# lucidrains/audiolm-pytorch

Hardware: NVIDIA H100
Metric: CoarseTransformer tokens/sec fwd+bwd seq2048 (higher is better)
Workload: dtype bf16

## Files before the change

### audiolm_pytorch_b200/_lib.py

```python
from __future__ import annotations

import ctypes as C
import os
from pathlib import Path

import torch

_PKG = Path(__file__).resolve().parent
LIB_PATH = _PKG / "libalm_b200.so"

P = C.c_void_p
I = C.c_int
L = C.c_int64
F = C.c_float
U32 = C.c_uint32
U64 = C.c_uint64
DROP = [F, U64, U32]

SIGNATURES: dict[str, list] = {
    "alm_gemm_bf16": [P, I, L, L, P, I, L, L, P, I, L, L, I, I, I, I, F, P, I, I, P],
    "alm_mqa_attn_fwd": [P, L, P, L, L, P, L, L, P, P, L, P, L, P, L, L, I, I, I, I, I, F, *DROP, P],
    "alm_mqa_attn_bwd": [P, L, P, L, L, P, L, L, P, L, P, P, P, I, P, L, P, P, L, P, L, P, P, L, L, I, I, I, I, I, F, *DROP,
                         P],
    "alm_pack_key_mask": [P, P, I, I, P],
# ... 22 lines not shown
    "alm_cast_pad_multi": [P, I, P],
    "alm_scale_by_scalar_bf16": [P, P, L, P],
    "alm_topk_gumbel_sample": [P, L, P, L, P, I, I, I, F, P],
    "alm_resid_ln_fwd": [P, P, P, P, P, P, P, I, I, P],
    "alm_resid_ln_bwd": [P, P, P, P, P, P, P, P, P, F, I, I, P],
    "alm_residual_unit_fwd": [P, P, P, P, P, P, I, I, I, I, I, P],
    "alm_causal_conv1d_fwd": [P, P, P, P, P, I, I, I, I, I, I, I, I, I, I, P],
    "alm_causal_convT1d_fwd": [P, P, P, P, I, I, I, I, I, P],
    "alm_codec_first_conv": [P, P, P, P, I, I, I, I, I, P],
    "alm_codec_ru_tc": [P, P, P, P, P, I, I, I, I, I, I, P],
    "alm_codec_conv_tc": [P, P, P, P, I, I, I, I, I, I, I, I, I, I, P],
    "alm_codec_pack_c8s": [P, P, I, I, I, P],
    "alm_codec_last_conv": [P, P, P, P, I, I, I, I, I, P],
    "alm_rvq_encode": [P, L, P, P, P, L, P, L, I, I, I, I, P],
    "alm_rvq_pack_codebooks": [P, P, P, L, I, P],
    "alm_rvq_prepare": [P, L, P, P, L, P, I, I, P],
    "alm_rvq_select": [P, L, P, P, P, P, L, P, P, L, I, I, I, I, P],
    "alm_rvq_decode": [P, L, P, P, L, I, I, I, I, P],
}


class AlmError(RuntimeError):
    pass


_lib = None


def load() -> C.CDLL:
    global _lib
    if _lib is not None:
        return _lib
    if not LIB_PATH.exists():
        raise AlmError(
            f"{LIB_PATH} not found. Build it with `python -m audiolm_pytorch_b200.build` "
            "(there is no CPU / PyTorch fallback for the hot path)."
        )
    lib = C.CDLL(str(LIB_PATH), mode=os.RTLD_LOCAL | os.RTLD_NOW)
    lib.alm_version.restype = I
    lib.alm_status_string.restype = C.c_char_p
    lib.alm_status_string.argtypes = [I]
    lib.alm_launch_count.restype = C.c_ulonglong
    lib.alm_reset_launch_count.restype = None
    lib.alm_decode_stack_scratch_bytes.restype = L
    lib.alm_decode_stack_scratch_bytes.argtypes = [I, I, I, I]
    lib.alm_gemm_head_ce_tiles.restype = I
    lib.alm_gemm_head_ce_tiles.argtypes = [I]
    lib.alm_decode_stack_grid.restype = I
    lib.alm_decode_stack_grid.argtypes = []
    lib.alm_decode_stack_plan.restype = I
    lib.alm_decode_stack_plan.argtypes = [I, I, I, I, I, P]
    lib.alm_decode_stack_trace_offset.restype = L
    lib.alm_decode_stack_trace_offset.argtypes = [I, I, I, I]
    for name, argtypes in SIGNATURES.items():
        fn = getattr(lib, name)
        fn.argtypes = argtypes
        fn.restype = I
    _lib = lib
    return lib


def ptr(t) -> int | None:
    if t is None:
        return None
    return t.data_ptr()


def stream_handle() -> int:
    return torch.cuda.current_stream().cuda_stream


def call(name: str, *args) -> None:
    lib = load()
    conv = []
    for a in args:
        if isinstance(a, torch.Tensor):
            if not a.is_cuda:
                raise AlmError(f"{name}: got a {a.device} tensor; the hot path has no CPU implementation")
            conv.append(a.data_ptr())
        else:
            conv.append(a)
    rc = getattr(lib, name)(*conv, stream_handle())
    if rc != 0:
        raise AlmError(f"{name} failed: {lib.alm_status_string(rc).decode()} ({rc})")


def launch_count() -> int:
    return int(load().alm_launch_count())


def reset_launch_count() -> None:
    load().alm_reset_launch_count()
```

### audiolm_pytorch_b200/csrc/attn_fwd_wgmma.cu

```cuda
#include "alm_common.cuh"
#include "ptx_sm90.cuh"

namespace alm {

constexpr int ATT_BM = 128;
constexpr int ATT_BN = 128;
constexpr int ATT_D = 64;
constexpr int ATT_KV_STAGES = 4;
constexpr int ATT_THREADS = 384;
constexpr int ATT_TILE_BYTES = 128 * 64 * 2;
constexpr int ATT_SMEM_BYTES = ATT_TILE_BYTES * (1 + 2 * ATT_KV_STAGES) + 256;

struct AttnFwdParams {
  __nv_bfloat16* o;
  float* lse;
  const uint32_t* kmask;
  int kb_stride;
  const float* bias;
  long long bias_hs, bias_rs;
  long long ldo, lse_stride;
  int b, h, n_q, n_k;
  int causal;
  float scale_log2;
  int n_q_pad;
  DropoutArgs drop;
};

__device__ __forceinline__ float att_ex2(float x) {
  float y;
  asm("ex2.approx.ftz.f32 %0, %1;" : "=f"(y) : "f"(x));
  return y;
}

__device__ __forceinline__ uint64_t attn_fwd_keep_bits(const DropoutArgs& d, uint32_t qrow, uint32_t kbase, int c_lane) {
  const uint32_t odd = qrow & 1u;
  uint64_t bits = 0;
#pragma unroll
  for (int kk = 0; kk < ATT_BN / 16; ++kk) {
    const uint32_t j0 = kbase + 16 * kk + c_lane;
    const uint4 own = dropout_draw(d, qrow, j0 + odd);
    const uint32_t ra = __shfl_xor_sync(0xffffffffu, odd ? own.x : own.y, 4);
    const uint32_t rb = __shfl_xor_sync(0xffffffffu, odd ? own.z : own.w, 4);
    const uint4 other = odd ? make_uint4(0u, ra, 0u, rb) : make_uint4(ra, 0u, rb, 0u);
#pragma unroll
    for (int c = 0; c < 2; ++c) {
      const uint4 dr = (uint32_t)c == odd ? own : other;
#pragma unroll
      for (int half = 0; half < 2; ++half)
#pragma unroll
        for (int h = 0; h < 2; ++h)
          if (dropout_pick(d, dr, qrow + 8 * h, j0 + 8 * half + c)) bits |= 1ull << (8 * kk + 4 * half + 2 * h + c);
    }
  }
  return bits;
}

template <bool HAS_BIAS, bool DROPOUT>
__global__ void __launch_bounds__(ATT_THREADS, 1)
mqa_attn_fwd_kernel(const __grid_constant__ CUtensorMap tmQ, const __grid_constant__ CUtensorMap tmK,
                    const __grid_constant__ CUtensorMap tmV, const AttnFwdParams p) {
  extern __shared__ __align__(1024) uint8_t smem_raw[];
  uint8_t* smem = smem_raw;
  if ((smem_u32(smem) & 1023u) != 0) __trap();
  uint8_t* sQ = smem;
  uint8_t* sK = sQ + ATT_TILE_BYTES;
  uint8_t* sV = sK + ATT_KV_STAGES * ATT_TILE_BYTES;
  uint64_t* bars = reinterpret_cast<uint64_t*>(sV + ATT_KV_STAGES * ATT_TILE_BYTES);
  uint64_t* q_full = bars;
  uint64_t* kv_full = bars + 1;
  uint64_t* kv_empty = kv_full + ATT_KV_STAGES;

  const int warp = threadIdx.x >> 5;
  const int lane = threadIdx.x & 31;
  const int wg = warp >> 2;
  const int n_qblocks = (p.n_q + ATT_BM - 1) / ATT_BM;
  const int qb = n_qblocks - 1 - (int)blockIdx.x;
  const int head = blockIdx.y;
  const int batch = blockIdx.z;
  const int q0 = qb * ATT_BM;
  const int off = p.n_k - p.n_q;
  int kv_end = p.n_k;
  if (p.causal) kv_end = min(p.n_k, q0 + ATT_BM + off);
  const int n_tiles = kv_end > 0 ? (kv_end + ATT_BN - 1) / ATT_BN : 0;

  if (threadIdx.x == 0) {
    tma_prefetch_desc(&tmQ);
    tma_prefetch_desc(&tmK);
    tma_prefetch_desc(&tmV);
    mbar_init(q_full, 1);
    for (int i = 0; i < ATT_KV_STAGES; ++i) {
      mbar_init(&kv_full[i], 1);
      mbar_init(&kv_empty[i], 8);
    }
    fence_mbar_init();
  }
  __syncthreads();

  if (wg == 0) {
    if (warp == 0 && n_tiles > 0) {
      if (elect_one_sync()) {
        mbar_arrive_expect_tx(q_full, ATT_TILE_BYTES);
        tma_load_3d(sQ, &tmQ, q_full, head * ATT_D, q0, batch);
      }
      __syncwarp();
      int stage = 0;
      uint32_t phase = 0;
      for (int j = 0; j < n_tiles; ++j) {
        mbar_wait(&kv_empty[stage], phase ^ 1u);
        if (elect_one_sync()) {
          mbar_arrive_expect_tx(&kv_full[stage], 2 * ATT_TILE_BYTES);
          tma_load_3d(sK + stage * ATT_TILE_BYTES, &tmK, &kv_full[stage], 0, j * ATT_BN, batch);
          tma_load_3d(sV + stage * ATT_TILE_BYTES, &tmV, &kv_full[stage], 0, j * ATT_BN, batch);
        }
        __syncwarp();
        if (++stage == ATT_KV_STAGES) { stage = 0; phase ^= 1u; }
      }
    }
    return;
  }

  const int cw = wg - 1;
  const int r_base = cw * 64 + (warp & 3) * 16 + (lane >> 2);
  const int c_lane = 2 * (lane & 3);
  constexpr float kLog2e = 1.4426950408889634f;
  float m_run[2] = {-INFINITY, -INFINITY}, l_run[2] = {0.f, 0.f};
  float o_acc[ATT_D / 2];
#pragma unroll
  for (int d = 0; d < ATT_D / 2; ++d) o_acc[d] = 0.f;
  int q_limit[2];
  [[maybe_unused]] const float* brow[2];
#pragma unroll
  for (int h = 0; h < 2; ++h) {
    const int qi = q0 + r_base + 8 * h;
    q_limit[h] = min(p.causal ? qi + off : p.n_k - 1, p.n_k - 1);
    if constexpr (HAS_BIAS) brow[h] = p.bias + (long long)head * p.bias_hs + (long long)min(qi, p.n_q - 1) * p.bias_rs;
  }
  const uint32_t* mrow = p.kmask ? p.kmask + (long long)batch * p.kb_stride : nullptr;
  const uint32_t q_addr = smem_u32(sQ) + cw * 8192;
  [[maybe_unused]] const uint32_t drop_row = ((uint32_t)batch * p.h + head) * (uint32_t)p.n_q_pad + q0 + r_base;

  if (n_tiles > 0) mbar_wait(q_full, 0);
  int stage = 0;
  uint32_t phase = 0;
  for (int j = 0; j < n_tiles; ++j) {
    mbar_wait(&kv_full[stage], phase);
    const uint32_t k_addr = smem_u32(sK + stage * ATT_TILE_BYTES);
    const uint32_t v_addr = smem_u32(sV + stage * ATT_TILE_BYTES);
    float s[ATT_BN / 2];
    wgmma_fence();
#pragma unroll
    for (int k = 0; k < ATT_D / 16; ++k)
      wgmma_ss<ATT_BN>(s, wgmma_desc_sw128(q_addr + k * 32, 1024, 16), wgmma_desc_sw128(k_addr + k * 32, 1024, 16),
                       k > 0 ? 1u : 0u);
    wgmma_commit();
    [[maybe_unused]] uint64_t keep = 0;
    if constexpr (DROPOUT) keep = attn_fwd_keep_bits(p.drop, drop_row, j * ATT_BN, c_lane);
    wgmma_wait<0>();
    wgmma_fence_acc(s);

    const int kbase = j * ATT_BN;
    const bool tile_full = mrow == nullptr && kbase + ATT_BN <= p.n_k && (!p.causal || kbase + ATT_BN - 1 <= q0 + off);
    uint32_t valid[4] = {0xFFFFFFFFu, 0xFFFFFFFFu, 0xFFFFFFFFu, 0xFFFFFFFFu};
    if (!tile_full && mrow != nullptr) {
      const uint4 mv = __ldg(reinterpret_cast<const uint4*>(mrow + j * 4));
      valid[0] = mv.x; valid[1] = mv.y; valid[2] = mv.z; valid[3] = mv.w;
    }
    uint32_t pa[ATT_BN / 16][4];
#pragma unroll
    for (int h = 0; h < 2; ++h) {
#pragma unroll
      for (int g = 0; g < ATT_BN / 8; ++g)
#pragma unroll
        for (int c = 0; c < 2; ++c) {
          const int col = 8 * g + c_lane + c;
          float v = s[4 * g + 2 * h + c] * p.scale_log2;
          if constexpr (HAS_BIAS) {
            if (kbase + col < p.bias_rs) v = fmaf(__ldg(brow[h] + kbase + col), kLog2e, v);
          }
          if (!tile_full) {
            const bool ok = kbase + col <= q_limit[h] && ((valid[col >> 5] >> (col & 31)) & 1u);
            if (!ok) v = -INFINITY;
          }
          s[4 * g + 2 * h + c] = v;
        }
      float m_tile = -INFINITY;
#pragma unroll
      for (int g = 0; g < ATT_BN / 8; ++g) m_tile = fmaxf(m_tile, fmaxf(s[4 * g + 2 * h], s[4 * g + 2 * h + 1]));
      m_tile = fmaxf(m_tile, __shfl_xor_sync(0xffffffffu, m_tile, 1));
      m_tile = fmaxf(m_tile, __shfl_xor_sync(0xffffffffu, m_tile, 2));
      const float m_new = fmaxf(m_run[h], m_tile);
      const float m_use = (m_new == -INFINITY) ? 0.f : m_new;
      const float alpha = att_ex2(m_run[h] - m_use);
      float l_tile = 0.f;
#pragma unroll
      for (int g = 0; g < ATT_BN / 8; ++g)
#pragma unroll
        for (int c = 0; c < 2; ++c) {
          const float pv = att_ex2(s[4 * g + 2 * h + c] - m_use);
          s[4 * g + 2 * h + c] = pv;
          l_tile += pv;
        }
      l_run[h] = fmaf(l_run[h], alpha, l_tile);
      m_run[h] = m_new;
#pragma unroll
      for (int g = 0; g < ATT_D / 8; ++g) {
        o_acc[4 * g + 2 * h] *= alpha;
        o_acc[4 * g + 2 * h + 1] *= alpha;
      }
    }
    if constexpr (DROPOUT) {
#pragma unroll
      for (int e = 0; e < ATT_BN / 2; ++e) s[e] = ((keep >> e) & 1u) ? s[e] * p.drop.scale : 0.f;
    }
#pragma unroll
    for (int kk = 0; kk < ATT_BN / 16; ++kk) {
      pa[kk][0] = pack_bf16x2(s[8 * kk + 0], s[8 * kk + 1]);
      pa[kk][1] = pack_bf16x2(s[8 * kk + 2], s[8 * kk + 3]);
      pa[kk][2] = pack_bf16x2(s[8 * kk + 4], s[8 * kk + 5]);
      pa[kk][3] = pack_bf16x2(s[8 * kk + 6], s[8 * kk + 7]);
    }
    wgmma_fence_acc(o_acc);
    wgmma_fence();
#pragma unroll
    for (int kk = 0; kk < ATT_BN / 16; ++kk)
      wgmma_rs<ATT_D, 1>(o_acc, pa[kk], wgmma_desc_sw128(v_addr + kk * 2048, 1024, 8192), 1u);
    wgmma_commit();
    wgmma_wait<0>();
    wgmma_fence_acc(o_acc);
    if (lane == 0) mbar_arrive(&kv_empty[stage]);
    if (++stage == ATT_KV_STAGES) { stage = 0; phase ^= 1u; }
  }

#pragma unroll
  for (int h = 0; h < 2; ++h) {
    float l_tot = l_run[h];
    l_tot += __shfl_xor_sync(0xffffffffu, l_tot, 1);
    l_tot += __shfl_xor_sync(0xffffffffu, l_tot, 2);
    const int qi = q0 + r_base + 8 * h;
    if (qi < p.n_q) {
      const float inv = l_tot > 0.f ? 1.f / l_tot : 0.f;
      __nv_bfloat16* dst = p.o + ((long long)batch * p.n_q + qi) * p.ldo + head * ATT_D + c_lane;
#pragma unroll
      for (int g = 0; g < ATT_D / 8; ++g)
        *reinterpret_cast<uint32_t*>(dst + 8 * g) = pack_bf16x2(o_acc[4 * g + 2 * h] * inv, o_acc[4 * g + 2 * h + 1] * inv);
      if (p.lse != nullptr && (lane & 3) == 0) {
        const float lse = l_tot > 0.f ? (m_run[h] + log2f(l_tot)) : INFINITY;
        p.lse[((long long)batch * p.h + head) * p.lse_stride + qi] = lse;
      }
    }
  }
}

}

namespace alm {
__global__ void pack_key_mask_kernel(const uint8_t* __restrict__ mask, uint32_t* __restrict__ bits, int n_k, int words) {
  const int b = blockIdx.y;
  const int w = blockIdx.x * (blockDim.x >> 5) + (threadIdx.x >> 5);
  if (w >= words) return;
  const int k = w * 32 + (threadIdx.x & 31);
  const bool on = k < n_k && mask[(long long)b * n_k + k] != 0;
  const uint32_t v = __ballot_sync(0xffffffffu, on);
  if ((threadIdx.x & 31) == 0) bits[(long long)b * words + w] = v;
}
}

extern "C" int alm_pack_key_mask(const void* key_mask, void* bits, int b, int n_k, alm_stream_t stream_) {
  using namespace alm;
  cudaStream_t stream = reinterpret_cast<cudaStream_t>(stream_);
  ALM_REQUIRE(key_mask && bits && b > 0 && n_k > 0, ALM_ERR_ARG);
  const int words = (n_k + 127) / 128 * 4;
  dim3 grid(ceil_div(words, 8), b);
  pack_key_mask_kernel<<<grid, 256, 0, stream>>>(reinterpret_cast<const uint8_t*>(key_mask),
                                                 reinterpret_cast<uint32_t*>(bits), n_k, words);
  ALM_CHECK_LAUNCH();
  ALM_LAUNCHED(1);
  return ALM_OK;
}

extern "C" int alm_mqa_attn_fwd(const void* q, int64_t ldq, const void* k, int64_t ldk, int64_t k_bstride,
                                const void* v, int64_t ldv, int64_t v_bstride, const void* key_mask, void* o,
                                int64_t ldo, float* lse, int64_t lse_stride, const float* bias, int64_t bias_hstride,
                                int64_t bias_rstride, int b, int h, int n_q, int n_k, int causal, float scale,
                                float dropout_p, uint64_t seed, uint32_t site, alm_stream_t stream_) {
  using namespace alm;
  cudaStream_t stream = reinterpret_cast<cudaStream_t>(stream_);
  ALM_REQUIRE(q && k && v && o, ALM_ERR_ARG);
  ALM_REQUIRE(b > 0 && h > 0 && n_q > 0 && n_k > 0 && n_k >= n_q, ALM_ERR_ARG);
  ALM_REQUIRE(dropout_p >= 0.f && dropout_p < 1.f, ALM_ERR_ARG);
  ALM_REQUIRE((long long)b * h * ((n_q + 127) / 128 * 128) < (1ll << 32), ALM_ERR_UNSUPPORTED);
  ALM_REQUIRE(ldq % 8 == 0 && ldk % 8 == 0 && ldv % 8 == 0 && ldo % 8 == 0, ALM_ERR_ALIGN);
  ALM_REQUIRE(k_bstride % 8 == 0 && v_bstride % 8 == 0, ALM_ERR_ALIGN);
  ALM_REQUIRE((reinterpret_cast<uintptr_t>(o) & 15u) == 0, ALM_ERR_ALIGN);
  if (bias != nullptr) {
    ALM_REQUIRE(bias_rstride >= n_k && bias_rstride % 4 == 0 && bias_hstride % 4 == 0, ALM_ERR_ALIGN);
    ALM_REQUIRE((reinterpret_cast<uintptr_t>(bias) & 15u) == 0, ALM_ERR_ALIGN);
  }

  CUtensorMap tmQ, tmK, tmV;
  {
    uint64_t dims[3] = {(uint64_t)h * ATT_D, (uint64_t)n_q, (uint64_t)b};
    uint64_t strides[3] = {2, (uint64_t)ldq * 2, (uint64_t)n_q * ldq * 2};
    uint32_t box[3] = {ATT_D, ATT_BM, 1};
    int rc = make_tensor_map(&tmQ, q, 2, 3, dims, strides, box, true);
    if (rc != ALM_OK) return rc;
  }
  {
    uint64_t dims[3] = {(uint64_t)ATT_D, (uint64_t)n_k, (uint64_t)b};
    uint64_t strides[3] = {2, (uint64_t)ldk * 2, (uint64_t)k_bstride * 2};
    uint32_t box[3] = {ATT_D, ATT_BN, 1};
    int rc = make_tensor_map(&tmK, k, 2, 3, dims, strides, box, true);
    if (rc != ALM_OK) return rc;
    strides[1] = (uint64_t)ldv * 2;
    strides[2] = (uint64_t)v_bstride * 2;
    rc = make_tensor_map(&tmV, v, 2, 3, dims, strides, box, true);
    if (rc != ALM_OK) return rc;
  }
  AttnFwdParams p;
  p.o = reinterpret_cast<__nv_bfloat16*>(o);
  p.lse = lse;
  p.kmask = reinterpret_cast<const uint32_t*>(key_mask);
  p.kb_stride = (n_k + 127) / 128 * 4;
  p.bias = bias;
  p.bias_hs = bias_hstride;
  p.bias_rs = bias_rstride;
  p.ldo = ldo;
  p.lse_stride = lse_stride;
  p.b = b; p.h = h; p.n_q = n_q; p.n_k = n_k;
  p.causal = causal;
  p.scale_log2 = scale * 1.4426950408889634f;
  p.n_q_pad = (n_q + 127) / 128 * 128;
  p.drop = make_dropout_args(dropout_p, seed, site);
  static bool attr_set = false;
  if (!attr_set) {
    ALM_CUDA_OK(cudaFuncSetAttribute(mqa_attn_fwd_kernel<false, false>, cudaFuncAttributeMaxDynamicSharedMemorySize,
                                     ATT_SMEM_BYTES));
    ALM_CUDA_OK(cudaFuncSetAttribute(mqa_attn_fwd_kernel<true, false>, cudaFuncAttributeMaxDynamicSharedMemorySize,
                                     ATT_SMEM_BYTES));
    ALM_CUDA_OK(cudaFuncSetAttribute(mqa_attn_fwd_kernel<false, true>, cudaFuncAttributeMaxDynamicSharedMemorySize,
                                     ATT_SMEM_BYTES));
    ALM_CUDA_OK(cudaFuncSetAttribute(mqa_attn_fwd_kernel<true, true>, cudaFuncAttributeMaxDynamicSharedMemorySize,
                                     ATT_SMEM_BYTES));
    attr_set = true;
  }
  dim3 grid((n_q + ATT_BM - 1) / ATT_BM, h, b);
  const bool drop = dropout_p > 0.f;
  if (bias != nullptr && drop)
    mqa_attn_fwd_kernel<true, true><<<grid, ATT_THREADS, ATT_SMEM_BYTES, stream>>>(tmQ, tmK, tmV, p);
  else if (bias != nullptr)
    mqa_attn_fwd_kernel<true, false><<<grid, ATT_THREADS, ATT_SMEM_BYTES, stream>>>(tmQ, tmK, tmV, p);
  else if (drop)
    mqa_attn_fwd_kernel<false, true><<<grid, ATT_THREADS, ATT_SMEM_BYTES, stream>>>(tmQ, tmK, tmV, p);
  else
    mqa_attn_fwd_kernel<false, false><<<grid, ATT_THREADS, ATT_SMEM_BYTES, stream>>>(tmQ, tmK, tmV, p);
  ALM_CHECK_LAUNCH();
  ALM_LAUNCHED(1);
  return ALM_OK;
}
```

### audiolm_pytorch_b200/ops.py

```python
from __future__ import annotations

import ctypes
import functools

import torch

from . import _lib

_SMS: dict[int, int] = {}


def num_sms(device=None) -> int:
    idx = None if device is None else torch.device(device).index
    if idx is None:
        idx = torch.cuda.current_device()
    if idx not in _SMS:
        _SMS[idx] = torch.cuda.get_device_properties(idx).multi_processor_count
    return _SMS[idx]


bf16 = torch.bfloat16
f32 = torch.float32


# ... 134 lines not shown
    bits = torch.empty(b, (n_k + 127) // 128 * 4, device=m.device, dtype=torch.int32)
    _lib.call("alm_pack_key_mask", m, bits, b, n_k)
    return PackedKeyMask(bits, n_k)


def _drop_args(dropout):
    if dropout is None:
        return 0.0, 0, 0
    p, seed, site = dropout
    if not 0.0 <= p < 1.0:
        raise ValueError(f"dropout probability must be in [0, 1), got {p}")
    return float(p), int(seed) & 0xFFFFFFFFFFFFFFFF, int(site) & 0xFFFFFFFF


def dropout_(x, p, seed, site):
    _check_cuda(x)
    assert x.dtype == bf16 and x.dim() == 2 and x.stride(1) == 1
    M, C = x.shape
    with _timed("dropout_bf16", M * C * 4, "byte"):
        _lib.call("alm_dropout_bf16", x, x.stride(0), M, C, *_drop_args((p, seed, site)))
    return x


def mqa_attn_fwd(q, k, v, *, heads, key_mask=None, causal=True, scale=None, return_lse=True, bias=None,
                 dropout=None):
    _check_cuda(q, k, v, bias)
    assert q.dtype == bf16 and k.dtype == bf16 and v.dtype == bf16
    b, n_q, hd = q.shape
    n_k = k.shape[1]
    assert hd == heads * 64 and k.shape[-1] == 64 and v.shape[-1] == 64, "dim_head must be 64"
    assert q.stride(-1) == 1 and k.stride(-1) == 1 and v.stride(-1) == 1
    assert q.stride(0) == n_q * q.stride(1)
    o = torch.empty(b, n_q, hd, device=q.device, dtype=bf16)
    n_q_pad = (n_q + 127) // 128 * 128
    lse = torch.empty(b, heads, n_q_pad, device=q.device, dtype=f32) if return_lse else None
    key_mask = pack_key_mask(key_mask)
    if key_mask is not None:
        assert key_mask.n_k == n_k and key_mask.bits.shape[0] == b
        key_mask = key_mask.bits
    if scale is None:
        scale = 64 ** -0.5
    vis = (n_q * n_k - n_q * (n_q - 1) / 2) if causal else n_q * n_k
    bhs, brs = _check_bias(bias, heads, n_q, n_k) if bias is not None else (0, 0)
    with _timed("mqa_attn_fwd_wgmma", 4.0 * b * heads * 64 * vis):
        _lib.call(
            "alm_mqa_attn_fwd",
            q, q.stride(1), k, k.stride(1), k.stride(0), v, v.stride(1), v.stride(0), key_mask,
            o, o.stride(1), lse, n_q_pad, bias, bhs, brs, b, heads, n_q, n_k, int(causal), float(scale),
            *_drop_args(dropout),
        )
    return o, lse


def mqa_attn_bwd(q, k, v, o, d_o, lse, *, heads, key_mask=None, causal=True, scale=None, bias=None, dbias=None,
                 dropout=None):
    _check_cuda(q, k, v, o, d_o, lse, bias, dbias)
    b, n_q, hd = q.shape
    n_k = k.shape[1]
    n_q_pad = lse.shape[-1]
    assert d_o.dtype == bf16 and d_o.stride(-1) == 1 and o.stride(-1) == 1
    assert d_o.stride(0) == n_q * d_o.stride(1)
    key_mask = pack_key_mask(key_mask)
    if key_mask is not None:
        assert key_mask.n_k == n_k
        key_mask = key_mask.bits
    if scale is None:
        scale = 64 ** -0.5
    dq = torch.empty(b, n_q, hd, device=q.device, dtype=bf16)
    delta = torch.empty(b, heads, n_q_pad, device=q.device, dtype=f32)
    dq_acc = torch.empty(b, n_q, hd, device=q.device, dtype=f32)
    dk = torch.empty(b, n_k, 64, device=q.device, dtype=bf16)
    dv = torch.empty(b, n_k, 64, device=q.device, dtype=bf16)
    bhs, brs = _check_bias(bias, heads, n_q, n_k) if bias is not None else (0, 0)
    if dbias is not None:
        assert bias is not None and dbias.dtype == f32 and dbias.shape == bias.shape and dbias.stride() == bias.stride()
    vis = (n_q * n_k - n_q * (n_q - 1) / 2) if causal else n_q * n_k
    with _timed("mqa_attn_bwd_wgmma", 10.0 * b * heads * 64 * vis):
        _lib.call("alm_attn_delta", o, o.stride(1), d_o, d_o.stride(1), delta, n_q_pad, dq_acc, b, heads, n_q)
        _lib.call(
            "alm_mqa_attn_bwd",
            q, q.stride(1), k, k.stride(1), k.stride(0), v, v.stride(1), v.stride(0), d_o, d_o.stride(1), key_mask,
            lse, delta, n_q_pad, dq, dq.stride(1), dq_acc, dk, dk.stride(1), dv, dv.stride(1),
            bias, dbias, bhs, brs, b, heads, n_q, n_k, int(causal), float(scale), *_drop_args(dropout),
        )
    return dq, dk, dv


def gemv(x, w, *, out_dtype=bf16, bias=None):
    _check_cuda(x, w, bias)
    rows, K = x.shape
    N = w.shape[0]
    assert x.dtype == bf16 and w.dtype == bf16 and x.stride(1) == 1 and w.stride(1) == 1 and rows <= 8
    assert w.shape[1] >= K and w.shape[1] % 8 == 0
    out = torch.empty(rows, N, device=x.device, dtype=out_dtype)
    _lib.call("alm_gemv_bf16", x, x.stride(0), w, w.stride(0), out, int(out_dtype == f32), out.stride(0),
              None if bias is None else bias.float().contiguous(), rows, N, K)
    return out


def kv_append(kv_new, k_cache, v_cache, cache_len):
    _check_cuda(kv_new, k_cache, v_cache, cache_len)
    b, max_len, dh = k_cache.shape
    assert dh == 64 and v_cache.shape == k_cache.shape and kv_new.shape == (b, 128) and kv_new.dtype == bf16
    assert k_cache.dtype == bf16 and v_cache.dtype == bf16 and cache_len.dtype == torch.int32
    assert k_cache.stride(1) == 64 and v_cache.stride() == k_cache.stride() and kv_new.stride(1) == 1
    _lib.call("alm_kv_append", kv_new, kv_new.stride(0), k_cache, v_cache, k_cache.stride(0), cache_len, max_len, b)
# ... 526 lines not shown
```

### include/alm_b200.h

```cpp
#ifndef ALM_B200_H_
#define ALM_B200_H_

#include <stddef.h>
#include <stdint.h>

#ifdef __cplusplus
extern "C" {
#endif

typedef struct CUstream_st* alm_stream_t;

typedef enum alm_status {
  ALM_OK = 0,
  ALM_ERR_ARG = -1,
  ALM_ERR_ALIGN = -2,
  ALM_ERR_CUDA = -3,
  ALM_ERR_UNSUPPORTED = -4
} alm_status;

int alm_version(void);
const char* alm_status_string(int code);
unsigned long long alm_launch_count(void);
void alm_reset_launch_count(void);

int alm_gemm_bf16(const void* A, int a_mn, int64_t lda, int64_t strideA, const void* B, int b_mn, int64_t ldb,
                  int64_t strideB, void* C, int c_fp32, int64_t ldc, int64_t strideC, int M, int N, int K, int batch,
                  float alpha, const float* bias, int acc_mode, int split_k, alm_stream_t stream);

int alm_embed_gather(const float* const* tables, int n_tables, const int32_t* src, float* out, int M, int d,
                     alm_stream_t stream);
int alm_embed_scatter(float* const* grad_tables, int n_tables, const int32_t* src, const float* dout, int M, int d,
                      alm_stream_t stream);
int alm_pack_key_mask(const void* key_mask, void* bits, int b, int n_k, alm_stream_t stream);
int alm_mqa_attn_fwd(const void* q, int64_t ldq, const void* k, int64_t ldk, int64_t k_bstride, const void* v,
                     int64_t ldv, int64_t v_bstride, const void* key_mask, void* o, int64_t ldo, float* lse,
                     int64_t lse_stride, const float* bias, int64_t bias_hstride, int64_t bias_rstride, int b, int h,
                     int n_q, int n_k, int causal, float scale, float dropout_p, uint64_t seed, uint32_t site,
                     alm_stream_t stream);

int alm_mqa_attn_bwd(const void* q, int64_t ldq, const void* k, int64_t ldk, int64_t k_bstride, const void* v,
                     int64_t ldv, int64_t v_bstride, const void* d_o, int64_t lddo, const void* key_mask,
                     const float* lse, const float* delta, int n_q_pad, void* dq, int64_t lddq, float* dq_acc,
                     void* dk, int64_t lddk, void* dv, int64_t lddv, const float* bias, float* dbias,
                     int64_t bias_hstride, int64_t bias_rstride, int b, int h, int n_q, int n_k, int causal,
                     float scale, float dropout_p, uint64_t seed, uint32_t site, alm_stream_t stream);
int alm_attn_delta(const void* o, int64_t ldo, const void* d_o, int64_t lddo, float* delta ,
                   int64_t delta_stride, float* dq_acc, int b, int h, int n, alm_stream_t stream);

int alm_bias_gather_fwd(const float* table, const int32_t* idx, const float* override_h, float* out, int heads,
                        int n_q, int n_k, int64_t ld, alm_stream_t stream);
int alm_bias_gather_bwd(const float* dbias, const int32_t* idx, float* dtable, float* doverride, int heads, int n_q,
                        int n_k, int64_t ld, alm_stream_t stream);

int alm_gemv_bf16(const void* x, int64_t ldx, const void* W, int64_t ldw, void* out, int c_fp32, int64_t ldo,
                  const float* bias, int rows, int N, int K, alm_stream_t stream);
int alm_kv_append(const void* kv_new, int64_t ld, void* k_cache, void* v_cache, int64_t cache_bstride,
                  const int32_t* len, int max_len, int b, alm_stream_t stream);
int alm_mqa_attn_decode(const void* q, int64_t ldq, const void* k_cache, const void* v_cache, int64_t cache_bstride,
                        const int32_t* len, int max_len, const void* key_mask, int64_t mask_bstride, const float* bias,
                        int64_t bias_ld, void* o, int64_t ldo,
                        float* workspace , int splits, int b, int h,
                        float scale, alm_stream_t stream);
int alm_decode_bias_row(const float* table, int rows, const float* override_h, const int32_t* u, const int32_t* cls,
                        int c, const int32_t* len, int max_len, float* out, int64_t ld, int h, alm_stream_t stream);

int alm_gemm_head_ce_tiles(int V);
int alm_gemm_head_ce(const void* X, int64_t ldx, const void* W, int64_t ldw, const float* bias, const int64_t* labels,
                     int64_t ignore_index, int mode, float* part, float* lab_logit, const float* lse,
                     const float* scale_num, const float* scale_den, void* dlogits, int64_t ldd, int M, int V, int K,
                     alm_stream_t stream);
int alm_ce_finish(const float* part, int tiles, const float* lab_logit, const int64_t* labels, int64_t ignore_index,
                  float* lse, float* loss_rows, int M, alm_stream_t stream);

int alm_decode_stack_grid(void);
int alm_decode_stack_plan(int b, int d, int heads, int inner, int n_layers, int32_t* staged);
int64_t alm_decode_stack_scratch_bytes(int b, int d, int heads, int inner);
int64_t alm_decode_stack_trace_offset(int b, int d, int heads, int inner);
int alm_decode_stack_step(const void* layer_table, int n_layers, const float* x, void* out, const float* final_gamma,
                          int32_t* len, int max_len, int64_t cache_bstride, const void* key_mask, int64_t mask_bstride,
                          void* scratch, int64_t scratch_bytes, int b, int d, int heads, int inner, int value_residual,
                          float scale, int grid_ctas , alm_stream_t stream);

int alm_hc_pre_fwd(const void* R_in, const void* Y, const float* beta_prev, const float* x_expand,
                   const float* gamma_hc, const float* dyn_alpha, const float* dyn_beta, const float* static_alpha,
                   const float* static_beta, const float* alpha_scale, const float* beta_scale,
                   const float* ln_gamma, void* R_out, void* bin, void* xn, float* beta_out, float* aux, int M,
                   int d, int streams, alm_stream_t stream);
int alm_hc_pre_bwd(const void* R_in, const void* Y, const float* beta_prev, const float* x_expand,
                   const float* gamma_hc, const float* dyn_alpha, const float* dyn_beta, const float* static_alpha,
                   const float* static_beta, const float* alpha_scale, const float* beta_scale,
                   const float* ln_gamma, const float* aux, const void* dR_out, const void* dxn,
// ... 74 lines not shown
```

Measured before the change: 746,100.

## Make attention forward persistent with double-buffered Q and S/PV wgmma overlap

Turns the attention forward kernel into a persistent kernel. A grid sized to the SM count walks over (batch, head, q-block) work items, and Q is double-buffered with empty/full barriers so the next item's Q loads while the current one computes. Inside an item, the loop is software-pipelined: the QK^T wgmma for the next KV tile is issued together with the PV wgmma for the current tile, with softmax running between the waits. It also adds setmaxnreg register rebalancing between producer and consumer warpgroups, mask-bit precomputation, a schedule query API and optional clock tracing, at the cost of a second Q buffer in shared memory and more register pressure.

Measured after the change: 761,600, median of 6. 1.02x the previous value.

```diff
diff --git a/audiolm_pytorch_b200/_lib.py b/audiolm_pytorch_b200/_lib.py
--- a/audiolm_pytorch_b200/_lib.py
+++ b/audiolm_pytorch_b200/_lib.py
@@ -98,6 +98,8 @@
     lib.alm_decode_stack_plan.argtypes = [I, I, I, I, I, P]
     lib.alm_decode_stack_trace_offset.restype = L
     lib.alm_decode_stack_trace_offset.argtypes = [I, I, I, I]
+    lib.alm_attn_fwd_schedule.restype = I
+    lib.alm_attn_fwd_schedule.argtypes = [I, I, I, I, I, I, P]
     for name, argtypes in SIGNATURES.items():
         fn = getattr(lib, name)
         fn.argtypes = argtypes
diff --git a/audiolm_pytorch_b200/csrc/attn_fwd_wgmma.cu b/audiolm_pytorch_b200/csrc/attn_fwd_wgmma.cu
--- a/audiolm_pytorch_b200/csrc/attn_fwd_wgmma.cu
+++ b/audiolm_pytorch_b200/csrc/attn_fwd_wgmma.cu
@@ -9,7 +9,7 @@
 constexpr int ATT_KV_STAGES = 4;
 constexpr int ATT_THREADS = 384;
 constexpr int ATT_TILE_BYTES = 128 * 64 * 2;
-constexpr int ATT_SMEM_BYTES = ATT_TILE_BYTES * (1 + 2 * ATT_KV_STAGES) + 256;
+constexpr int ATT_SMEM_BYTES = ATT_TILE_BYTES * (2 + 2 * ATT_KV_STAGES) + 256;
 
 struct AttnFwdParams {
   __nv_bfloat16* o;
@@ -26,6 +26,23 @@
   DropoutArgs drop;
 };
 
+struct AttnFwdItem {
+  int batch, head, qb, n_tiles;
+};
+__host__ __device__ __forceinline__ AttnFwdItem attn_fwd_item(int i, int b, int h, int n_q, int n_k, int causal) {
+  const int n_qblocks = (n_q + ATT_BM - 1) / ATT_BM;
+  const int bh = i % (b * h);
+  AttnFwdItem w;
+  w.qb = n_qblocks - 1 - i / (b * h);
+  w.batch = bh / h;
+  w.head = bh - w.batch * h;
+  const int kv_end = causal ? min(n_k, (w.qb + 1) * ATT_BM + n_k - n_q) : n_k;
+  w.n_tiles = (kv_end + ATT_BN - 1) / ATT_BN;
+  return w;
+}
+inline int attn_fwd_items(int b, int h, int n_q) { return b * h * ((n_q + ATT_BM - 1) / ATT_BM); }
+inline int attn_fwd_grid(int n_items, int n_sm) { return n_items < n_sm ? n_items : n_sm; }
+
 __device__ __forceinline__ float att_ex2(float x) {
   float y;
   asm("ex2.approx.ftz.f32 %0, %1;" : "=f"(y) : "f"(x));
@@ -54,6 +71,18 @@
   }
   return bits;
 }
+
+constexpr int AF_TRACE_ITERS = 64, AF_TRACE_STAMPS = 8;
+#ifdef ALM_ATTN_FWD_TRACE
+__device__ long long g_attn_fwd_trace[2][AF_TRACE_ITERS][AF_TRACE_STAMPS];
+#define AF_STAMP(i)                                                                                   \
+  do {                                                                                                \
+    if (blockIdx.x == 0 && (threadIdx.x & 127) == 0 && tt < AF_TRACE_ITERS)                           \
+      g_attn_fwd_trace[(threadIdx.x >> 7) - 1][tt][i] = clock64();                                    \
+  } while (0)
+#else
+#define AF_STAMP(i)
+#endif
 
 template <bool HAS_BIAS, bool DROPOUT>
 __global__ void __launch_bounds__(ATT_THREADS, 1)
@@ -63,31 +92,27 @@
   uint8_t* smem = smem_raw;
   if ((smem_u32(smem) & 1023u) != 0) __trap();
   uint8_t* sQ = smem;
-  uint8_t* sK = sQ + ATT_TILE_BYTES;
+  uint8_t* sK = sQ + 2 * ATT_TILE_BYTES;
   uint8_t* sV = sK + ATT_KV_STAGES * ATT_TILE_BYTES;
   uint64_t* bars = reinterpret_cast<uint64_t*>(sV + ATT_KV_STAGES * ATT_TILE_BYTES);
   uint64_t* q_full = bars;
-  uint64_t* kv_full = bars + 1;
+  uint64_t* q_empty = bars + 2;
+  uint64_t* kv_full = bars + 4;
   uint64_t* kv_empty = kv_full + ATT_KV_STAGES;
 
   const int warp = threadIdx.x >> 5;
   const int lane = threadIdx.x & 31;
   const int wg = warp >> 2;
-  const int n_qblocks = (p.n_q + ATT_BM - 1) / ATT_BM;
-  const int qb = n_qblocks - 1 - (int)blockIdx.x;
-  const int head = blockIdx.y;
-  const int batch = blockIdx.z;
-  const int q0 = qb * ATT_BM;
-  const int off = p.n_k - p.n_q;
-  int kv_end = p.n_k;
-  if (p.causal) kv_end = min(p.n_k, q0 + ATT_BM + off);
-  const int n_tiles = kv_end > 0 ? (kv_end + ATT_BN - 1) / ATT_BN : 0;
+  const int n_items = p.b * p.h * ((p.n_q + ATT_BM - 1) / ATT_BM);
 
   if (threadIdx.x == 0) {
     tma_prefetch_desc(&tmQ);
     tma_prefetch_desc(&tmK);
     tma_prefetch_desc(&tmV);
-    mbar_init(q_full, 1);
+    for (int i = 0; i < 2; ++i) {
+      mbar_init(&q_full[i], 1);
+      mbar_init(&q_empty[i], 8);
+    }
     for (int i = 0; i < ATT_KV_STAGES; ++i) {
       mbar_init(&kv_full[i], 1);
       mbar_init(&kv_empty[i], 8);
@@ -97,155 +122,242 @@
   __syncthreads();
 
   if (wg == 0) {
-    if (warp == 0 && n_tiles > 0) {
-      if (elect_one_sync()) {
-        mbar_arrive_expect_tx(q_full, ATT_TILE_BYTES);
-        tma_load_3d(sQ, &tmQ, q_full, head * ATT_D, q0, batch);
-      }
-      __syncwarp();
+    setmaxnreg_dec<24>();
+    if (warp == 0) {
       int stage = 0;
       uint32_t phase = 0;
-      for (int j = 0; j < n_tiles; ++j) {
-        mbar_wait(&kv_empty[stage], phase ^ 1u);
+      int it = 0;
+      for (int item = blockIdx.x; item < n_items; item += gridDim.x, ++it) {
+        const AttnFwdItem w = attn_fwd_item(item, p.b, p.h, p.n_q, p.n_k, p.causal);
+        const int qbuf = it & 1;
+        mbar_wait(&q_empty[qbuf], ((it >> 1) & 1) ^ 1u);
         if (elect_one_sync()) {
-          mbar_arrive_expect_tx(&kv_full[stage], 2 * ATT_TILE_BYTES);
-          tma_load_3d(sK + stage * ATT_TILE_BYTES, &tmK, &kv_full[stage], 0, j * ATT_BN, batch);
-          tma_load_3d(sV + stage * ATT_TILE_BYTES, &tmV, &kv_full[stage], 0, j * ATT_BN, batch);
+          mbar_arrive_expect_tx(&q_full[qbuf], ATT_TILE_BYTES);
+          tma_load_3d(sQ + qbuf * ATT_TILE_BYTES, &tmQ, &q_full[qbuf], w.head * ATT_D, w.qb * ATT_BM, w.batch);
         }
         __syncwarp();
-        if (++stage == ATT_KV_STAGES) { stage = 0; phase ^= 1u; }
+        for (int j = 0; j < w.n_tiles; ++j) {
+          mbar_wait(&kv_empty[stage], phase ^ 1u);
+          if (elect_one_sync()) {
+            mbar_arrive_expect_tx(&kv_full[stage], 2 * ATT_TILE_BYTES);
+            tma_load_3d(sK + stage * ATT_TILE_BYTES, &tmK, &kv_full[stage], 0, j * ATT_BN, w.batch);
+            tma_load_3d(sV + stage * ATT_TILE_BYTES, &tmV, &kv_full[stage], 0, j * ATT_BN, w.batch);
+          }
+          __syncwarp();
+          if (++stage == ATT_KV_STAGES) { stage = 0; phase ^= 1u; }
+        }
       }
     }
     return;
   }
 
+  setmaxnreg_inc<240>();
   const int cw = wg - 1;
   const int r_base = cw * 64 + (warp & 3) * 16 + (lane >> 2);
   const int c_lane = 2 * (lane & 3);
   constexpr float kLog2e = 1.4426950408889634f;
-  float m_run[2] = {-INFINITY, -INFINITY}, l_run[2] = {0.f, 0.f};
-  float o_acc[ATT_D / 2];
-#pragma unroll
-  for (int d = 0; d < ATT_D / 2; ++d) o_acc[d] = 0.f;
-  int q_limit[2];
-  [[maybe_unused]] const float* brow[2];
-#pragma unroll
-  for (int h = 0; h < 2; ++h) {
-    const int qi = q0 + r_base + 8 * h;
-    q_limit[h] = min(p.causal ? qi + off : p.n_k - 1, p.n_k - 1);
-    if constexpr (HAS_BIAS) brow[h] = p.bias + (long long)head * p.bias_hs + (long long)min(qi, p.n_q - 1) * p.bias_rs;
-  }
-  const uint32_t* mrow = p.kmask ? p.kmask + (long long)batch * p.kb_stride : nullptr;
-  const uint32_t q_addr = smem_u32(sQ) + cw * 8192;
-  [[maybe_unused]] const uint32_t drop_row = ((uint32_t)batch * p.h + head) * (uint32_t)p.n_q_pad + q0 + r_base;
-
-  if (n_tiles > 0) mbar_wait(q_full, 0);
+  const int off = p.n_k - p.n_q;
   int stage = 0;
   uint32_t phase = 0;
-  for (int j = 0; j < n_tiles; ++j) {
+  [[maybe_unused]] int tt = 0;
+  int it = 0;
+  for (int item = blockIdx.x; item < n_items; item += gridDim.x, ++it) {
+    const AttnFwdItem w = attn_fwd_item(item, p.b, p.h, p.n_q, p.n_k, p.causal);
+    const int q0 = w.qb * ATT_BM;
+    float m_run[2] = {-INFINITY, -INFINITY}, l_run[2] = {0.f, 0.f};
+    float o_acc[ATT_D / 2];
+#pragma unroll
+    for (int d = 0; d < ATT_D / 2; ++d) o_acc[d] = 0.f;
+    int q_limit[2];
+    [[maybe_unused]] const float* brow[2];
+#pragma unroll
+    for (int h = 0; h < 2; ++h) {
+      const int qi = q0 + r_base + 8 * h;
+      q_limit[h] = min(p.causal ? qi + off : p.n_k - 1, p.n_k - 1);
+      if constexpr (HAS_BIAS)
+        brow[h] = p.bias + (long long)w.head * p.bias_hs + (long long)min(qi, p.n_q - 1) * p.bias_rs;
+    }
+    const uint32_t* mrow = p.kmask ? p.kmask + (long long)w.batch * p.kb_stride : nullptr;
+    const uint32_t q_addr = smem_u32(sQ + (it & 1) * ATT_TILE_BYTES) + cw * 8192;
+    [[maybe_unused]] const uint32_t drop_row = ((uint32_t)w.batch * p.h + w.head) * (uint32_t)p.n_q_pad + q0 + r_base;
+
+    float s[ATT_BN / 2];
+    uint32_t pa[ATT_BN / 16][4];
+    float alpha[2];
+
+    auto issue_s = [&](int st) {
+      const uint32_t k_addr = smem_u32(sK + st * ATT_TILE_BYTES);
+#pragma unroll
+      for (int k = 0; k < ATT_D / 16; ++k)
+        wgmma_ss<ATT_BN>(s, wgmma_desc_sw128(q_addr + k * 32, 1024, 16), wgmma_desc_sw128(k_addr + k * 32, 1024, 16),
+                         k > 0 ? 1u : 0u);
+      wgmma_commit();
+    };
+    auto load_mask = [&](int jj) {
+      return mrow != nullptr ? __ldg(reinterpret_cast<const uint4*>(mrow + jj * 4))
+                             : make_uint4(0xFFFFFFFFu, 0xFFFFFFFFu, 0xFFFFFFFFu, 0xFFFFFFFFu);
+    };
+    auto softmax = [&](int jj, uint4 mv) {
+      const int kbase = jj * ATT_BN;
+      const bool tile_full = mrow == nullptr && kbase + ATT_BN <= p.n_k && (!p.causal || kbase + ATT_BN - 1 <= q0 + off);
+      uint32_t vis[2][4];
+#pragma unroll
+      for (int h = 0; h < 2; ++h) {
+        const int lim = q_limit[h] - kbase;
+        const uint32_t valid[4] = {mv.x, mv.y, mv.z, mv.w};
+#pragma unroll
+        for (int wd = 0; wd < 4; ++wd) {
+          const int n = min(max(lim + 1 - 32 * wd, 0), 32);
+          const uint32_t lead = n == 32 ? 0xFFFFFFFFu : (1u << n) - 1u;
+          vis[h][wd] = (valid[wd] & lead) >> c_lane;
+        }
+      }
+      float m_use[2];
+#pragma unroll
+      for (int h = 0; h < 2; ++h) {
+#pragma unroll
+        for (int g = 0; g < ATT_BN / 8; ++g)
+#pragma unroll
+          for (int c = 0; c < 2; ++c) {
+            float v = s[4 * g + 2 * h + c];
+            if constexpr (HAS_BIAS) {
+              const int col = 8 * g + c_lane + c;
+              v *= p.scale_log2;
+              if (kbase + col < p.bias_rs) v = fmaf(__ldg(brow[h] + kbase + col), kLog2e, v);
+            }
+            if (HAS_BIAS && !tile_full && !((vis[h][g >> 2] >> (8 * (g & 3) + c)) & 1u)) v = -INFINITY;
+            s[4 * g + 2 * h + c] = v;
+          }
+        if (!HAS_BIAS && !tile_full) {
+#pragma unroll
+          for (int g = 0; g < ATT_BN / 8; ++g)
+#pragma unroll
+            for (int c = 0; c < 2; ++c)
+              if (!((vis[h][g >> 2] >> (8 * (g & 3) + c)) & 1u)) s[4 * g + 2 * h + c] = -INFINITY;
+        }
+        float m_tile = -INFINITY;
+#pragma unroll
+        for (int g = 0; g < ATT_BN / 8; ++g) m_tile = fmaxf(m_tile, fmaxf(s[4 * g + 2 * h], s[4 * g + 2 * h + 1]));
+        m_tile = fmaxf(m_tile, __shfl_xor_sync(0xffffffffu, m_tile, 1));
+        m_tile = fmaxf(m_tile, __shfl_xor_sync(0xffffffffu, m_tile, 2));
+        if constexpr (!HAS_BIAS) m_tile *= p.scale_log2;
+        const float m_new = fmaxf(m_run[h], m_tile);
+        m_use[h] = (m_new == -INFINITY) ? 0.f : m_new;
+        alpha[h] = att_ex2(m_run[h] - m_use[h]);
+        m_run[h] = m_new;
+      }
+      AF_STAMP(3);
+#pragma unroll
+      for (int h = 0; h < 2; ++h) {
+        float l_tile = 0.f;
+#pragma unroll
+        for (int g = 0; g < ATT_BN / 8; ++g)
+#pragma unroll
+          for (int c = 0; c < 2; ++c) {
+            const float x = s[4 * g + 2 * h + c];
+            const float pv = HAS_BIAS ? att_ex2(x - m_use[h]) : att_ex2(fmaf(x, p.scale_log2, -m_use[h]));
+            s[4 * g + 2 * h + c] = pv;
+            l_tile += pv;
+          }
+        l_run[h] = fmaf(l_run[h], alpha[h], l_tile);
+      }
+      AF_STAMP(4);
+    };
+    auto pack = [&](uint64_t keep) {
+      if constexpr (DROPOUT) {
+#pragma unroll
+        for (int e = 0; e < ATT_BN / 2; ++e) s[e] = ((keep >> e) & 1u) ? s[e] * p.drop.scale : 0.f;
+      }
+#pragma unroll
+      for (int kk = 0; kk < ATT_BN / 16; ++kk) {
+        pa[kk][0] = pack_bf16x2(s[8 * kk + 0], s[8 * kk + 1]);
+        pa[kk][1] = pack_bf16x2(s[8 * kk + 2], s[8 * kk + 3]);
+        pa[kk][2] = pack_bf16x2(s[8 * kk + 4], s[8 * kk + 5]);
+        pa[kk][3] = pack_bf16x2(s[8 * kk + 6], s[8 * kk + 7]);
+      }
+    };
+    auto issue_pv = [&](int st) {
+      const uint32_t v_addr = smem_u32(sV + st * ATT_TILE_BYTES);
+#pragma unroll
+      for (int kk = 0; kk < ATT_BN / 16; ++kk)
+        wgmma_rs<ATT_D, 1>(o_acc, pa[kk], wgmma_desc_sw128(v_addr + kk * 2048, 1024, 8192), 1u);
+      wgmma_commit();
+    };
+    [[maybe_unused]] uint64_t keep = 0;
+
+    uint4 mask_next = load_mask(0);
+    mbar_wait(&q_full[it & 1], (it >> 1) & 1);
     mbar_wait(&kv_full[stage], phase);
-    const uint32_t k_addr = smem_u32(sK + stage * ATT_TILE_BYTES);
-    const uint32_t v_addr = smem_u32(sV + stage * ATT_TILE_BYTES);
-    float s[ATT_BN / 2];
     wgmma_fence();
-#pragma unroll
-    for (int k = 0; k < ATT_D / 16; ++k)
-      wgmma_ss<ATT_BN>(s, wgmma_desc_sw128(q_addr + k * 32, 1024, 16), wgmma_desc_sw128(k_addr + k * 32, 1024, 16),
-                       k > 0 ? 1u : 0u);
-    wgmma_commit();
-    [[maybe_unused]] uint64_t keep = 0;
-    if constexpr (DROPOUT) keep = attn_fwd_keep_bits(p.drop, drop_row, j * ATT_BN, c_lane);
+    issue_s(stage);
+    if constexpr (DROPOUT) keep = attn_fwd_keep_bits(p.drop, drop_row, 0, c_lane);
     wgmma_wait<0>();
     wgmma_fence_acc(s);
-
-    const int kbase = j * ATT_BN;
-    const bool tile_full = mrow == nullptr && kbase + ATT_BN <= p.n_k && (!p.causal || kbase + ATT_BN - 1 <= q0 + off);
-    uint32_t valid[4] = {0xFFFFFFFFu, 0xFFFFFFFFu, 0xFFFFFFFFu, 0xFFFFFFFFu};
-    if (!tile_full && mrow != nullptr) {
-      const uint4 mv = __ldg(reinterpret_cast<const uint4*>(mrow + j * 4));
-      valid[0] = mv.x; valid[1] = mv.y; valid[2] = mv.z; valid[3] = mv.w;
-    }
-    uint32_t pa[ATT_BN / 16][4];
-#pragma unroll
-    for (int h = 0; h < 2; ++h) {
-#pragma unroll
-      for (int g = 0; g < ATT_BN / 8; ++g)
-#pragma unroll
-        for (int c = 0; c < 2; ++c) {
-          const int col = 8 * g + c_lane + c;
-          float v = s[4 * g + 2 * h + c] * p.scale_log2;
-          if constexpr (HAS_BIAS) {
-            if (kbase + col < p.bias_rs) v = fmaf(__ldg(brow[h] + kbase + col), kLog2e, v);
-          }
-          if (!tile_full) {
-            const bool ok = kbase + col <= q_limit[h] && ((valid[col >> 5] >> (col & 31)) & 1u);
-            if (!ok) v = -INFINITY;
-          }
-          s[4 * g + 2 * h + c] = v;
-        }
-      float m_tile = -INFINITY;
-#pragma unroll
-      for (int g = 0; g < ATT_BN / 8; ++g) m_tile = fmaxf(m_tile, fmaxf(s[4 * g + 2 * h], s[4 * g + 2 * h + 1]));
-      m_tile = fmaxf(m_tile, __shfl_xor_sync(0xffffffffu, m_tile, 1));
-      m_tile = fmaxf(m_tile, __shfl_xor_sync(0xffffffffu, m_tile, 2));
-      const float m_new = fmaxf(m_run[h], m_tile);
-      const float m_use = (m_new == -INFINITY) ? 0.f : m_new;
-      const float alpha = att_ex2(m_run[h] - m_use);
-      float l_tile = 0.f;
-#pragma unroll
-      for (int g = 0; g < ATT_BN / 8; ++g)
-#pragma unroll
-        for (int c = 0; c < 2; ++c) {
-          const float pv = att_ex2(s[4 * g + 2 * h + c] - m_use);
-          s[4 * g + 2 * h + c] = pv;
-          l_tile += pv;
-        }
-      l_run[h] = fmaf(l_run[h], alpha, l_tile);
-      m_run[h] = m_new;
-#pragma unroll
-      for (int g = 0; g < ATT_D / 8; ++g) {
-        o_acc[4 * g + 2 * h] *= alpha;
-        o_acc[4 * g + 2 * h + 1] *= alpha;
-      }
-    }
-    if constexpr (DROPOUT) {
-#pragma unroll
-      for (int e = 0; e < ATT_BN / 2; ++e) s[e] = ((keep >> e) & 1u) ? s[e] * p.drop.scale : 0.f;
-    }
-#pragma unroll
-    for (int kk = 0; kk < ATT_BN / 16; ++kk) {
-      pa[kk][0] = pack_bf16x2(s[8 * kk + 0], s[8 * kk + 1]);
-      pa[kk][1] = pack_bf16x2(s[8 * kk + 2], s[8 * kk + 3]);
-      pa[kk][2] = pack_bf16x2(s[8 * kk + 4], s[8 * kk + 5]);
-      pa[kk][3] = pack_bf16x2(s[8 * kk + 6], s[8 * kk + 7]);
+    softmax(0, mask_next);
+    pack(keep);
+
+    for (int j = 0; j + 1 < w.n_tiles; ++j) {
+      AF_STAMP(0);
+      if constexpr (!DROPOUT) mask_next = load_mask(j + 1);
+      const int cur = stage;
+      if (++stage == ATT_KV_STAGES) { stage = 0; phase ^= 1u; }
+      mbar_wait(&kv_full[stage], phase);
+      AF_STAMP(1);
+      wgmma_fence_acc(o_acc);
+      wgmma_fence();
+      issue_s(stage);
+      issue_pv(cur);
+      if constexpr (DROPOUT) {
+        keep = attn_fwd_keep_bits(p.drop, drop_row, (j + 1) * ATT_BN, c_lane);
+        mask_next = load_mask(j + 1);
+      }
+      wgmma_wait<1>();
+      wgmma_fence_acc(s);
+      AF_STAMP(2);
+      softmax(j + 1, mask_next);
+      wgmma_wait<0>();
+      wgmma_fence_acc(o_acc);
+#pragma unroll
+      for (int h = 0; h < 2; ++h)
+#pragma unroll
+        for (int g = 0; g < ATT_D / 8; ++g) {
+          o_acc[4 * g + 2 * h] *= alpha[h];
+          o_acc[4 * g + 2 * h + 1] *= alpha[h];
+        }
+      AF_STAMP(5);
+      pack(keep);
+      AF_STAMP(6);
+      if (lane == 0) mbar_arrive(&kv_empty[cur]);
+      AF_STAMP(7);
+      ++tt;
     }
     wgmma_fence_acc(o_acc);
     wgmma_fence();
-#pragma unroll
-    for (int kk = 0; kk < ATT_BN / 16; ++kk)
-      wgmma_rs<ATT_D, 1>(o_acc, pa[kk], wgmma_desc_sw128(v_addr + kk * 2048, 1024, 8192), 1u);
-    wgmma_commit();
+    issue_pv(stage);
     wgmma_wait<0>();
     wgmma_fence_acc(o_acc);
     if (lane == 0) mbar_arrive(&kv_empty[stage]);
     if (++stage == ATT_KV_STAGES) { stage = 0; phase ^= 1u; }
-  }
-
-#pragma unroll
-  for (int h = 0; h < 2; ++h) {
-    float l_tot = l_run[h];
-    l_tot += __shfl_xor_sync(0xffffffffu, l_tot, 1);
-    l_tot += __shfl_xor_sync(0xffffffffu, l_tot, 2);
-    const int qi = q0 + r_base + 8 * h;
-    if (qi < p.n_q) {
-      const float inv = l_tot > 0.f ? 1.f / l_tot : 0.f;
-      __nv_bfloat16* dst = p.o + ((long long)batch * p.n_q + qi) * p.ldo + head * ATT_D + c_lane;
-#pragma unroll
-      for (int g = 0; g < ATT_D / 8; ++g)
-        *reinterpret_cast<uint32_t*>(dst + 8 * g) = pack_bf16x2(o_acc[4 * g + 2 * h] * inv, o_acc[4 * g + 2 * h + 1] * inv);
-      if (p.lse != nullptr && (lane & 3) == 0) {
-        const float lse = l_tot > 0.f ? (m_run[h] + log2f(l_tot)) : INFINITY;
-        p.lse[((long long)batch * p.h + head) * p.lse_stride + qi] = lse;
+    ++tt;
+    if (lane == 0) mbar_arrive(&q_empty[it & 1]);
+
+#pragma unroll
+    for (int h = 0; h < 2; ++h) {
+      float l_tot = l_run[h];
+      l_tot += __shfl_xor_sync(0xffffffffu, l_tot, 1);
+      l_tot += __shfl_xor_sync(0xffffffffu, l_tot, 2);
+      const int qi = q0 + r_base + 8 * h;
+      if (qi < p.n_q) {
+        const float inv = l_tot > 0.f ? 1.f / l_tot : 0.f;
+        __nv_bfloat16* dst = p.o + ((long long)w.batch * p.n_q + qi) * p.ldo + w.head * ATT_D + c_lane;
+#pragma unroll
+        for (int g = 0; g < ATT_D / 8; ++g)
+          *reinterpret_cast<uint32_t*>(dst + 8 * g) =
+              pack_bf16x2(o_acc[4 * g + 2 * h] * inv, o_acc[4 * g + 2 * h + 1] * inv);
+        if (p.lse != nullptr && (lane & 3) == 0) {
+          const float lse = l_tot > 0.f ? (m_run[h] + log2f(l_tot)) : INFINITY;
+          p.lse[((long long)w.batch * p.h + w.head) * p.lse_stride + qi] = lse;
+        }
       }
     }
   }
@@ -287,7 +399,7 @@
   cudaStream_t stream = reinterpret_cast<cudaStream_t>(stream_);
   ALM_REQUIRE(q && k && v && o, ALM_ERR_ARG);
   ALM_REQUIRE(b > 0 && h > 0 && n_q > 0 && n_k > 0 && n_k >= n_q, ALM_ERR_ARG);
-  ALM_REQUIRE(dropout_p >= 0.f && dropout_p < 1.f, ALM_ERR_ARG);
+  ALM_REQUIRE(dropout_p >= 0.f && dropout_p < 1.f && scale > 0.f, ALM_ERR_ARG);
   ALM_REQUIRE((long long)b * h * ((n_q + 127) / 128 * 128) < (1ll << 32), ALM_ERR_UNSUPPORTED);
   ALM_REQUIRE(ldq % 8 == 0 && ldk % 8 == 0 && ldv % 8 == 0 && ldo % 8 == 0, ALM_ERR_ALIGN);
   ALM_REQUIRE(k_bstride % 8 == 0 && v_bstride % 8 == 0, ALM_ERR_ALIGN);
@@ -343,7 +455,7 @@
                                      ATT_SMEM_BYTES));
     attr_set = true;
   }
-  dim3 grid((n_q + ATT_BM - 1) / ATT_BM, h, b);
+  const int grid = attn_fwd_grid(attn_fwd_items(b, h, n_q), num_sms());
   const bool drop = dropout_p > 0.f;
   if (bias != nullptr && drop)
     mqa_attn_fwd_kernel<true, true><<<grid, ATT_THREADS, ATT_SMEM_BYTES, stream>>>(tmQ, tmK, tmV, p);
@@ -357,3 +469,24 @@
   ALM_LAUNCHED(1);
   return ALM_OK;
 }
+
+extern "C" int alm_attn_fwd_schedule(int b, int h, int n_q, int n_k, int causal, int n_sm, int32_t* items) {
+  using namespace alm;
+  ALM_REQUIRE(b > 0 && h > 0 && n_q > 0 && n_k >= n_q && n_sm > 0, ALM_ERR_ARG);
+  const int n_items = attn_fwd_items(b, h, n_q);
+  for (int i = 0; items != nullptr && i < n_items; ++i) {
+    const AttnFwdItem w = attn_fwd_item(i, b, h, n_q, n_k, causal);
+    items[4 * i] = w.batch;
+    items[4 * i + 1] = w.head;
+    items[4 * i + 2] = w.qb;
+    items[4 * i + 3] = w.n_tiles;
+  }
+  return attn_fwd_grid(n_items, n_sm);
+}
+
+#ifdef ALM_ATTN_FWD_TRACE
+extern "C" int alm_attn_fwd_trace_read(long long* dst) {
+  ALM_CUDA_OK(cudaMemcpyFromSymbol(dst, alm::g_attn_fwd_trace, sizeof(alm::g_attn_fwd_trace)));
+  return ALM_OK;
+}
+#endif
diff --git a/audiolm_pytorch_b200/ops.py b/audiolm_pytorch_b200/ops.py
--- a/audiolm_pytorch_b200/ops.py
+++ b/audiolm_pytorch_b200/ops.py
@@ -210,6 +210,15 @@
     return o, lse
 
 
+def attn_fwd_schedule(b, heads, n_q, n_k, causal, n_sm):
+    n_items = b * heads * (-(-n_q // 128))
+    items = torch.empty(n_items, 4, dtype=torch.int32)
+    grid = _lib.load().alm_attn_fwd_schedule(b, heads, n_q, n_k, int(causal), n_sm, items.data_ptr())
+    if grid <= 0:
+        raise _lib.AlmError(f"alm_attn_fwd_schedule failed ({grid})")
+    return grid, items
+
+
 def mqa_attn_bwd(q, k, v, o, d_o, lse, *, heads, key_mask=None, causal=True, scale=None, bias=None, dbias=None,
                  dropout=None):
     _check_cuda(q, k, v, o, d_o, lse, bias, dbias)
diff --git a/include/alm_b200.h b/include/alm_b200.h
--- a/include/alm_b200.h
+++ b/include/alm_b200.h
@@ -37,6 +37,7 @@
                      int64_t lse_stride, const float* bias, int64_t bias_hstride, int64_t bias_rstride, int b, int h,
                      int n_q, int n_k, int causal, float scale, float dropout_p, uint64_t seed, uint32_t site,
                      alm_stream_t stream);
+int alm_attn_fwd_schedule(int b, int h, int n_q, int n_k, int causal, int n_sm, int32_t* items);
 
 int alm_mqa_attn_bwd(const void* q, int64_t ldq, const void* k, int64_t ldk, int64_t k_bstride, const void* v,
                      int64_t ldv, int64_t v_bstride, const void* d_o, int64_t lddo, const void* key_mask,
```
